# disanda/Deep-GAN-Encoders

Hardware: AMD Instinct MI355X
Metric: encoder-train images/sec (E_align_s2 step, StyleGAN2 FFHQ-1024) (higher is better)
Workload: dtype bf16; 1 GPU; E_align_s2 two-phase step, StyleGAN2-1024 G (train mode) + BE(startf=16, L=9) + LPIPS-VGG16 (seeded stand-in weights), batch 8/GPU; global_batch=8, img_size=1024, parallelism=dp1

## Files before the change

deep-gan-encoders_amd/_lib.py:

```python
import ctypes as C
import os

_HERE = os.path.dirname(os.path.abspath(__file__))
LIB_PATH = os.environ.get("DGE_LIB_PATH", os.path.join(_HERE, "libdge_hip.so"))


class DgeError(RuntimeError):
    pass


class ConvDesc(C.Structure):
    _fields_ = [
        ("x", C.c_void_p), ("w_packed", C.c_void_p), ("y", C.c_void_p), ("addend", C.c_void_p), ("dot_src", C.c_void_p),
        ("in_scale", C.c_void_p), ("in_shift", C.c_void_p), ("out_scale", C.c_void_p),
        ("bias", C.c_void_p), ("noise", C.c_void_p), ("noise_w", C.c_void_p), ("stats", C.c_void_p),
        ("B", C.c_int), ("H", C.c_int), ("W", C.c_int), ("Cin", C.c_int), ("Cout", C.c_int),
        ("ksize", C.c_int), ("up", C.c_int), ("in_s2d", C.c_int), ("noise_batch", C.c_int), ("noise_w_per_channel", C.c_int),
        ("act", C.c_int), ("bias_scale", C.c_float), ("gain", C.c_float), ("add_scale", C.c_float),
        ("dtype", C.c_int), ("in_up2", C.c_int), ("in_relu", C.c_int), ("stats_slots", C.c_int), ("w_layout", C.c_int),
        ("prep", C.c_int), ("prep_gain", C.c_float), ("prep_noise", C.c_void_p), ("prep_ns", C.c_void_p), ("prep_noise_batch", C.c_int),
        ("prep_stats", C.c_void_p), ("mask_relu", C.c_int), ("in_t2d", C.c_int),
        ("rgb_w", C.c_void_p), ("rgb_style", C.c_void_p), ("rgb_bias", C.c_void_p), ("rgb_out", C.c_void_p), ("rgb_wscale", C.c_float),
        ("rgb_skip_y", C.c_int), ("pool_out", C.c_int), ("pool_mask", C.c_void_p),
        ("prefetch_w", C.c_void_p), ("prefetch_ntot", C.c_int), ("prefetch_cin", C.c_int), ("in_bwd_coef", C.c_void_p),
# ... 37 lines not shown
    "dge_torgb_bwd_prep": [_P, _P, _P, _P, _P, _P, _I, _P, _P, _P, _I, _I, _I, _F, _F, _I, _P],
    "dge_demod_bwd_prep": [_P, _I, _P, _P, _P, _I, _I, _F, _P],
    "dge_sum_slots": [_P, _P, _I, _I, _I, _P],
    "dge_sum_slots_planar": [_P, _P, _I, _I, _I, _P],
    "dge_set_deterministic": [_I],
    "dge_get_deterministic": [],
    "dge_packed_n": [_I],
    "dge_pack_conv_weight": [_P, _P, _I, _I, _I, _I, _I, _F, _P],
    "dge_pack_conv_weights_multi": [_P, _P, _I, _I, _P],
    "dge_pack_desc_bytes": [],
    "dge_weight_sumsq": [_P, _P, _I, _I, _I, _F, _P],
    "dge_linear": [_P, _I, _P, _P, _P, _I, _I, _I, _I, _F, _F, _F, _I, _F, _I, _P],
    "dge_pixelnorm": [_P, _P, _I, _I, _F, _P],
    "dge_truncation": [_P, _P, _P, _I, _I, _I, _F, _I, _I, _P],
    "dge_torgb": [_P, _P, _P, _P, _P, _P, _I, _I, _I, _I, _F, _I, _P],
    "dge_conv_rgb_supported": [_I, _I, _I, _I, _I, _I, _I],
    "dge_conv_in_bwd_supported": [_I, _I, _I, _I, _I, _I, _I],
    "dge_conv_in_bwd_fromrgb_supported": [_I, _I, _I, _I, _I, _I, _I],
    "dge_conv_in_bwd_x_supported": [_I, _I, _I, _I, _I, _I, _I],
    "dge_conv_pool_supported": [_I, _I, _I, _I, _I, _I, _I],
    "dge_rgb_upsample_add": [_P, _P, _I, _I, _I, _P],
    "dge_nchw_to_nhwc": [_P, _P, _I, _I, _I, _I, _I, _P],
    "dge_nhwc_to_nchw": [_P, _P, _I, _I, _I, _I, _P],
    "dge_fromrgb": [_P, _P, _P, _P, _P, _I, _I, _I, _I, _P],
    "dge_fromrgb2": [_P, _P, _P, _P, _P, _P, _I, _I, _I, _I, _P],
    "dge_stats_finalize": [_P, _P, _P, _P, _I, _I, _I, _F, _P],
    "dge_stats_finalize_slots": [_P, _I, _P, _P, _P, _I, _I, _I, _F, _P],
    "dge_blend": [_P, _P, _P, _P, _P, _P, _I, _I, _I, _I, _I, _F, _F, _I, _P],
    "dge_loss_reduce": [_P, _P, _P, _I, _I, _I, _I, _I, _I, _I, _I, _P],
    "dge_crop_pool": [_P, _P, _I, _I, _I, _I, _I, _I, _I, _I, _P],
    "dge_ssim_fwd": [_P, _P, _P, _P, _I, _I, _I, _P],
    "dge_ssim_box7": [_P, _P, _P, _I, _I, _I, _F, _F, _F, _P],
    "dge_ssim_bwd": [_P, _P, _P, _P, _I, _I, _I, _F, _I, _P],
    "dge_space_loss_finalize": [_P, _P, _P, _P, _F, _F, _I, _P],
    "dge_space_loss_bwd": [_P, _P, _P, _P, _P, _I, _I, _I, _I, _I, _I, _I, _I, _F, _F, _I, _P],
    "dge_axpy_scalar": [_P, _P, _P, C.c_long, _F, _I, _P],
    "dge_lreq_adam_multi": [_I, _P, _P, _P, _P, _P, _F, _F, _P, _P, _P],
    "dge_modconv_bwd_prep": [_P, _P, _P, _P, _P, _P, _I, _I, _I, _I, _F, _I, _P],
    "dge_demod_bwd": [_P, _P, _P, _P, _P, _I, _I, _F, _P],
    "dge_linear_t": [_P, _I, _I, _P, _P, _P, _I, _I, _I, _I, _I, _F, _I, _P],
    "dge_torgb_bwd": [_P, _P, _P, _P, _P, _P, _I, _I, _I, _F, _I, _P],
    "dge_up2_bwd": [_P, _P, _I, _I, _I, _P],
    "dge_conv_wgrad": [_P, _P, _P, _P, _P, _I, _I, _I, _I, _I, _I, _I, _P],
    "dge_act_bwd": [_P, _P, _P, _P, _P, _I, _I, _I, _I, _I, _I, _F, _F, _I, _P],
    "dge_in_bwd_coef": [_P, _P, _P, _P, _P, _P, _I, _I, _I, _P],
    "dge_in_bwd_coef_slots": [_P, _I, _P, _P, _P, _P, _P, _I, _I, _I, _P],
    "dge_in_bwd": [_P, _P, _P, _P, _P, _P, _P, _I, _I, _I, _I, _I, _F, _I, _I, _P],
    "dge_chan_sum": [_P, _P, _I, _I, _I, _F, _I, _P],
    "dge_fromrgb_bwd": [_P, _P, _P, _P, _I, _I, _I, _I, _P],
    "dge_head_entry_size": [],
    "dge_heads_bwd": [_P, _I, _I, _P, _I, _P, _P, _P, _P, _I, _I, _P],
    "dge_dense_wgrad": [_P, _I, _P, _I, _P, _P, _I, _I, _I, _I, _P],
    "dge_lpips_prep": [_P, _P, _I, _I, _I, _P, _P, _I, _P],
    "dge_lpips_prep_bwd": [_P, _P, _I, _I, _I, _P, _F, _I, _I, _P],
    "dge_maxpool2": [_P, _P, _I, _I, _I, _I, _I, _P],
    "dge_maxpool2_bwd": [_P, _P, _P, _P, _I, _I, _I, _I, _I, _P],
    "dge_lpips_head": [_P, _P, _P, _P, _I, _I, _I, _F, _I, _P],
    "dge_mean": [_P, _P, _I, _P],
    "dge_blur_noise_act": [_P, _P, _P, _P, _P, _P, _I, _I, _I, _I, _I, _I, _I, _I, _P],
    "dge_affine_compose": [_P, _P, _P, _P, _P, _I, _I, _P],
    "dge_lerp_layers": [_P, _P, _I, _P, _P, _I, _I, _I, _P],
    "dge_linear_rows": [_P, _I, _P, _P, _P, _P, _P, _P, _I, _I, _I, _F, _F, _F, _P],
    "dge_demod_rows": [_P, _P, _P, _P, _P, _P, _P, _P, _I, _I, _F, _P],
    "dge_fromrgb_dgrad": [_P, _P, _P, _P, _I, _I, _I, _I, _P],
    "dge_nearest_up2": [_P, _P, _I, _I, _I, _I, _F, _I, _P],
    "dge_sg1_in_bwd_coef": [_P, _P, _P, _P, _P, _P, _I, _I, _I, _P],
# ... 93 lines not shown
```

deep-gan-encoders_amd/csrc/loss_kernels.hip:

```cpp
#include "common.h"
#include "../../include/dge_hip.h"

struct Crop { int H, W, y0, x0, h, w; };

__device__ __forceinline__ void block_atomic_sums(float* vals, int n, float* out, float* red) {
    const int lane = threadIdx.x & 63, wave = threadIdx.x >> 6;
    for (int i = 0; i < n; i++) {
        const float s = wave_sum(vals[i]);
        if (lane == 0) red[i * 4 + wave] = s;
    }
    __syncthreads();
    if (det_on()) {
        const int nslots = gridDim.x;
        float* slot = det_slot(0, 1, blockIdx.x, nslots, 8);
        if (threadIdx.x < n) slot[threadIdx.x] = red[threadIdx.x * 4] + red[threadIdx.x * 4 + 1] + red[threadIdx.x * 4 + 2] + red[threadIdx.x * 4 + 3];
        if (det_arrive_wg(0, nslots)) {
            __shared__ float dred[16];
            for (int i = 0; i < n; i++) {
                const float t = det_total_wg(0, nslots, 8, i, dred);
                if (threadIdx.x == 0) out[i] += t;
            }
        }
        return;
    }
// ... 12 lines not shown
        float ma = -INFINITY, mb = -INFINITY;
        for (int c = 0; c < C; c++) {
            const float av = a[off + c * plane], bv = b[off + c * plane];
            const float d = av - bv;
            v[0] += d * d; v[1] += av * bv; v[2] += av * av; v[3] += bv * bv; v[4] += av; v[5] += bv;
            ma = fmaxf(ma, av); mb = fmaxf(mb, bv);
        }
        float sa = 0.f, sb = 0.f;
        for (int c = 0; c < C; c++) { sa += __expf(a[off + c * plane] - ma); sb += __expf(b[off + c * plane] - mb); }
        const float lsa = __logf(sa) + ma, lsb = __logf(sb) + mb;
        for (int c = 0; c < C; c++) {
            const float la = a[off + c * plane] - lsa, lb = b[off + c * plane] - lsb;
            v[6] += __expf(la) * (la - lb);
        }
    }
    block_atomic_sums(v, 7, sums, red);
}

__global__ void crop_pool_kernel(const float* __restrict__ src, float* __restrict__ dst, int BC, Crop cr, int k) {
    const int oh = cr.h / k, ow = cr.w / k;
    const long n = (long)BC * oh * ow;
    const long idx = blockIdx.x * 256L + threadIdx.x;
    if (idx >= n) return;
    const int x = idx % ow; const long r = idx / ow; const int y = r % oh; const int bc = r / oh;
    const float* p = src + (size_t)bc * cr.H * cr.W + (size_t)(cr.y0 + y * k) * cr.W + cr.x0 + x * k;
    float s = 0.f;
    for (int i = 0; i < k; i++)
        for (int j = 0; j < k; j++) s += p[(size_t)i * cr.W + j];
    dst[idx] = s / (float)(k * k);
}

struct Gauss11 { float g[11]; };

__global__ __launch_bounds__(256) void ssim_fwd_kernel(const float* __restrict__ a, const float* __restrict__ b,
                                                        float* __restrict__ ssim_sum, float* __restrict__ dmap,
                                                        int BC, int h, int w, Gauss11 G) {
    __shared__ float ta[26][27], tb[26][27];
    __shared__ float red[4];
    const int bc = blockIdx.z, x0 = blockIdx.x * 16, y0 = blockIdx.y * 16;
    const float* pa = a + (size_t)bc * h * w; const float* pb = b + (size_t)bc * h * w;
    for (int i = threadIdx.x; i < 26 * 26; i += 256) {
        const int ty = i / 26, tx = i % 26, gy = y0 + ty - 5, gx = x0 + tx - 5;
        const bool in = gy >= 0 && gy < h && gx >= 0 && gx < w;
        ta[ty][tx] = in ? pa[(size_t)gy * w + gx] : 0.f;
        tb[ty][tx] = in ? pb[(size_t)gy * w + gx] : 0.f;
    }
    __syncthreads();
    const int lx = threadIdx.x % 16, ly = threadIdx.x / 16, gx = x0 + lx, gy = y0 + ly;
    float S = 0.f;
    if (gx < w && gy < h) {
        float mu1 = 0, mu2 = 0, e11 = 0, e22 = 0, e12 = 0;
        for (int i = 0; i < 11; i++)
            for (int j = 0; j < 11; j++) {
                const float wgt = G.g[i] * G.g[j];
                const float av = ta[ly + i][lx + j], bv = tb[ly + i][lx + j];
                mu1 += wgt * av; mu2 += wgt * bv; e11 += wgt * av * av; e22 += wgt * bv * bv; e12 += wgt * av * bv;
            }
        const float C1 = 1e-4f, C2 = 9e-4f;
        const float s11 = e11 - mu1 * mu1, s22 = e22 - mu2 * mu2, s12 = e12 - mu1 * mu2;
        const float A1 = 2 * mu1 * mu2 + C1, A2 = 2 * s12 + C2, B1 = mu1 * mu1 + mu2 * mu2 + C1, B2 = s11 + s22 + C2;
        const float inv = 1.f / (B1 * B2);
        S = A1 * A2 * inv;
        if (dmap) {
            const size_t n = (size_t)BC * h * w, o = (size_t)bc * h * w + (size_t)gy * w + gx;
            dmap[o] = (2 * mu1 * A2 - 2 * mu1 * A1) * inv - S * (2 * mu2 / B1 - 2 * mu2 / B2);
            dmap[n + o] = -S / B2;
            dmap[2 * n + o] = 2 * A1 * inv;
        }
    }
    S = wave_sum(S);
    if ((threadIdx.x & 63) == 0) red[threadIdx.x >> 6] = S;
    __syncthreads();
    if (det_on()) {
        const int nslots = gridDim.x * gridDim.y * gridDim.z;
        const int sl = blockIdx.x + gridDim.x * (blockIdx.y + gridDim.y * blockIdx.z);
        float* slot = det_slot(0, 1, sl, nslots, 1);
        if (threadIdx.x == 0) slot[0] = red[0] + red[1] + red[2] + red[3];
        if (det_arrive_wg(0, nslots)) {
            __shared__ float dred[16];
            const float t = det_total_wg(0, nslots, 1, 0, dred);
            if (threadIdx.x == 0) ssim_sum[0] += t;
        }
        return;
    }
    if (threadIdx.x == 0) atomicAdd(ssim_sum + ((blockIdx.x + blockIdx.y * 7 + blockIdx.z * 13) & 31), red[0] + red[1] + red[2] + red[3]);
}

__global__ __launch_bounds__(256) void ssim_bwd_kernel(const float* __restrict__ a, const float* __restrict__ b,
                                                        const float* __restrict__ dmap, float* __restrict__ g,
                                                        int BC, int h, int w, Gauss11 G, float scale, int accumulate) {
    __shared__ float t0[26][27], t1[26][27], t2[26][27];
    const int bc = blockIdx.z, x0 = blockIdx.x * 16, y0 = blockIdx.y * 16;
    const size_t n = (size_t)BC * h * w, po = (size_t)bc * h * w;
    for (int i = threadIdx.x; i < 26 * 26; i += 256) {
        const int ty = i / 26, tx = i % 26, gy = y0 + ty - 5, gx = x0 + tx - 5;
        const bool in = gy >= 0 && gy < h && gx >= 0 && gx < w;
        const size_t o = po + (size_t)gy * w + gx;
        t0[ty][tx] = in ? dmap[o] : 0.f; t1[ty][tx] = in ? dmap[n + o] : 0.f; t2[ty][tx] = in ? dmap[2 * n + o] : 0.f;
    }
    __syncthreads();
    const int lx = threadIdx.x % 16, ly = threadIdx.x / 16, gx = x0 + lx, gy = y0 + ly;
    if (gx >= w || gy >= h) return;
    float f0 = 0, f1 = 0, f2 = 0;
    for (int i = 0; i < 11; i++)
        for (int j = 0; j < 11; j++) {
            const float wgt = G.g[i] * G.g[j];
            f0 += wgt * t0[ly + i][lx + j]; f1 += wgt * t1[ly + i][lx + j]; f2 += wgt * t2[ly + i][lx + j];
        }
    const size_t o = po + (size_t)gy * w + gx;
    const float v = scale * (f0 + 2.f * b[o] * f1 + a[o] * f2);
    g[o] = accumulate ? g[o] + v : v;
}

__global__ void space_loss_finalize_kernel(const float* __restrict__ sums, const float* __restrict__ ssim_sum,
                                           const float* __restrict__ lpips, float* __restrict__ out, float n, float n_pooled,
                                           int image_space) {
    if (threadIdx.x != 0 || blockIdx.x != 0) return;
    const float mse = sums[0] / n;
    const float cosv = 1.f - sums[1] / (sqrtf(sums[2]) * sqrtf(sums[3]));
    const float ma = sums[4] / n, mb = sums[5] / n;
    const float va = fmaxf((sums[2] - n * ma * ma) / (n - 1.f), 0.f), vb = fmaxf((sums[3] - n * mb * mb) / (n - 1.f), 0.f);
    const float dm = ma - mb, ds = sqrtf(va) - sqrtf(vb);
    float kl = sums[6] / n;
    if (isnan(kl)) kl = 0.f;
    if (isinf(kl)) kl = 1.f;
    float ssim_tot = 0.f;
    if (image_space) for (int k = 0; k < 32; k++) ssim_tot += ssim_sum[k];
    const float ssim_l = image_space ? 1.f - ssim_tot / n_pooled : 0.f;
    const float lp = (image_space && lpips) ? lpips[0] : 0.f;
    out[0] = 5.f * mse + 3.f * cosv + ssim_l + 2.f * lp;
    out[1] = mse; out[2] = dm * dm; out[3] = ds * ds; out[4] = kl; out[5] = cosv; out[6] = ssim_l; out[7] = lp;
}

__global__ void space_loss_bwd_kernel(const float* __restrict__ a, const float* __restrict__ b,
                                      const float* __restrict__ sums, const float* __restrict__ gp, float* __restrict__ g,
                                      int BC, Crop cr, int k, float n, float wgt, int accumulate) {
    const long tot = (long)BC * cr.h * cr.w;
    const long idx = blockIdx.x * 256L + threadIdx.x;
    if (idx >= tot) return;
    const int x = idx % cr.w; const long r = idx / cr.w; const int y = r % cr.h; const int bc = r / cr.h;
    const size_t off = (size_t)bc * cr.H * cr.W + (size_t)(cr.y0 + y) * cr.W + cr.x0 + x;
    const float na = sqrtf(sums[2]), nb = sqrtf(sums[3]);
    const float av = a[off], bv = b[off];
    float v = 10.f * (bv - av) / n + 3.f * (-av / (na * nb) + sums[1] * bv / (na * nb * nb * nb));
// ... 410 lines not shown
        const float inv = 1.f / 49.f, cn = 49.f / 48.f;
        const float ux = sx * inv, uy = sy * inv;
        const float vx = cn * (sxx * inv - ux * ux), vy = cn * (syy * inv - uy * uy), vxy = cn * (sxy * inv - ux * uy);
        const float C1 = (0.01f * R) * (0.01f * R), C2 = (0.03f * R) * (0.03f * R);
        S = ((2 * ux * uy + C1) * (2 * vxy + C2)) / ((ux * ux + uy * uy + C1) * (vx + vy + C2));
    }
    S = wave_sum(S);
    if ((threadIdx.x & 63) == 0) red[threadIdx.x >> 6] = S;
    __syncthreads();
    if (det_on()) {
        const int nslots = gridDim.x * gridDim.y, sl = blockIdx.x + gridDim.x * blockIdx.y;
        float* slot = det_slot(bc, gridDim.z, sl, nslots, 1);
        if (threadIdx.x == 0) slot[0] = red[0] + red[1] + red[2] + red[3];
        if (det_arrive_wg(bc, nslots)) {
            __shared__ float dred[16];
            const float t = det_total_wg(bc, nslots, 1, 0, dred);
            if (threadIdx.x == 0) sums[bc] += t;
        }
        return;
    }
    if (threadIdx.x == 0) atomicAdd(sums + bc, red[0] + red[1] + red[2] + red[3]);
}

extern "C" int dge_ssim_box7(const float* a, const float* b, float* sums, int BC, int h, int w, float scale, float shift, float data_range,
                             hipStream_t s) {
    DGE_CHECK(BC >= 1 && h >= 7 && w >= 7 && data_range > 0.f, "ssim_box7: planes must be at least 7x7 (got %dx%d)", h, w);
    hipLaunchKernelGGL(ssim_box7_kernel, dim3((w - 6 + 15) / 16, (h - 6 + 15) / 16, BC), dim3(256), 0, s, a, b, sums, h, w, scale, shift,
                       data_range);
    DGE_LAUNCH_CHECK("ssim_box7");
    return 0;
}

extern "C" int dge_ssim_fwd(const float* a, const float* b, float* ssim_sum, float* dmap, int BC, int h, int w, hipStream_t s) {
    hipLaunchKernelGGL(ssim_fwd_kernel, dim3((w + 15) / 16, (h + 15) / 16, BC), dim3(256), 0, s, a, b, ssim_sum, dmap, BC, h, w, gauss11());
    DGE_LAUNCH_CHECK("ssim_fwd");
    return 0;
}

extern "C" int dge_ssim_bwd(const float* a, const float* b, const float* dmap, float* g, int BC, int h, int w, float scale,
                            int accumulate, hipStream_t s) {
    hipLaunchKernelGGL(ssim_bwd_kernel, dim3((w + 15) / 16, (h + 15) / 16, BC), dim3(256), 0, s, a, b, dmap, g, BC, h, w, gauss11(), scale, accumulate);
    DGE_LAUNCH_CHECK("ssim_bwd");
    return 0;
}

extern "C" int dge_space_loss_finalize(const float* sums7, const float* ssim_sum, const float* lpips, float* out8, float n,
                                       float n_pooled, int image_space, hipStream_t s) {
    hipLaunchKernelGGL(space_loss_finalize_kernel, dim3(1), dim3(64), 0, s, sums7, ssim_sum, lpips, out8, n, n_pooled, image_space);
    DGE_LAUNCH_CHECK("space_loss_finalize");
    return 0;
}

extern "C" int dge_space_loss_bwd(const float* a, const float* b, const float* sums7, const float* g_pooled, float* g,
                                  int BC, int H, int W, int y0, int x0, int h, int w, int k, float n, float weight,
                                  int accumulate, hipStream_t s) {
    const long tot = (long)BC * h * w;
    hipLaunchKernelGGL(space_loss_bwd_kernel, dim3((unsigned)((tot + 255) / 256)), dim3(256), 0, s, a, b, sums7, g_pooled, g, BC,
                       mk(H, W, y0, x0, h, w), k, n, weight, accumulate);
    DGE_LAUNCH_CHECK("space_loss_bwd");
    return 0;
}

extern "C" int dge_axpy_scalar(const float* x, const float* scalar, float* y, long n, float extra, int accumulate, hipStream_t s) {
    hipLaunchKernelGGL(axpy_scalar_kernel, dim3((unsigned)((n + 255) / 256)), dim3(256), 0, s, x, scalar, y, n, extra, accumulate);
    DGE_LAUNCH_CHECK("axpy_scalar");
    return 0;
}
```

deep-gan-encoders_amd/losses.py:

```python
import contextlib
import os

import torch

from . import ops
from ._lib import lib, check
from .collectives import all_reduce
from .ops import _f32, _p, _stream


class GlobalBatch:

    def __init__(self, world):
        self.world = world

    def reduce(self, t):
        all_reduce(t)
        return t


def _pool_factor(h):
    k = 1
    while h > 256:
        h //= 2
        k *= 2
    return k


def attention_windows(H, W):
    oy, ox = H // 8 + H // 32, W // 8 + W // 32
    return [(0, 0, H, W), (0, W // 8, H, W - 2 * (W // 8)), (oy, ox, H - 2 * oy, W - 2 * ox)]


_PK = 48


def _window_reduce(a, b, win, image_space, lpips_model, need_grad, pk, world):
    B, Cc, H, W = a.shape
    y0, x0, h, w = win
    dev = a.device
    L = lib()
    slots = ops.zeros((16, 8), dev)
    check(L.dge_loss_reduce(_f32(a), _f32(b), _p(slots), B, Cc, H, W, y0, x0, h, w, _stream()), "dge_loss_reduce")
    ops._sum_over_batch(slots, pk[0:8])
    st = dict(win=win, pk=pk, k=1, npool=1.0, n=float(B * Cc * h * w) * world, lp=None, ap=None)
    if image_space:
        k = _pool_factor(h)
        hp, wp = h // k, w // k
        ap = torch.empty((B, Cc, hp, wp), dtype=torch.float32, device=dev)
        bp = torch.empty_like(ap)
        check(L.dge_crop_pool(_f32(a), _p(ap), B * Cc, H, W, y0, x0, h, w, k, _stream()), "dge_crop_pool")
        check(L.dge_crop_pool(_f32(b), _p(bp), B * Cc, H, W, y0, x0, h, w, k, _stream()), "dge_crop_pool")
        dmap = torch.empty((3, B, Cc, hp, wp), dtype=torch.float32, device=dev) if need_grad else None
        check(L.dge_ssim_fwd(_p(ap), _p(bp), _p(pk[8:40]), _p(dmap), B * Cc, hp, wp, _stream()), "dge_ssim_fwd")
        st.update(k=k, npool=float(B * Cc * hp * wp) * world, ap=ap, bp=bp, dmap=dmap, g_lp=None)
        if lpips_model is not None:
            lp, st["g_lp"] = lpips_model.value_and_grad(ap, bp, need_grad=need_grad)
            if world > 1:
                check(L.dge_axpy_scalar(_p(lp), None, _p(pk[40:41]), 1, 1.0 / world, 0, _stream()), "dge_axpy_scalar")
                lp = pk[40:41]
            st["lp"] = lp
    return st


def _window_finish(a, b, st, image_space, weight, g_out, accumulate, world):
    B, Cc, H, W = a.shape
    y0, x0, h, w = st["win"]
    dev = a.device
    L = lib()
    pk = st["pk"]
    out8 = torch.empty(8, dtype=torch.float32, device=dev)
    gp = None
    if image_space and g_out is not None:
        bp = st["bp"]
        gp = torch.empty_like(bp)
        check(L.dge_ssim_bwd(_p(st["ap"]), _p(bp), _p(st["dmap"]), _p(gp), B * Cc, bp.shape[2], bp.shape[3], -1.0 / st["npool"], 0,
                             _stream()), "dge_ssim_bwd")
        if st["g_lp"] is not None:
            check(L.dge_axpy_scalar(_p(st["g_lp"]), None, _p(gp), gp.numel(), 2.0 / world, 1, _stream()), "dge_axpy_scalar")
    check(L.dge_space_loss_finalize(_p(pk[0:8]), _p(pk[8:40]) if image_space else None, _p(st["lp"]), _p(out8), st["n"], st["npool"],
                                    1 if image_space else 0, _stream()), "dge_space_loss_finalize")
    if g_out is not None:
        check(L.dge_space_loss_bwd(_f32(a), _f32(b), _p(pk[0:8]), _p(gp), _p(g_out), B * Cc, H, W, y0, x0, h, w, st["k"], st["n"],
                                   float(weight), 1 if accumulate else 0, _stream()), "dge_space_loss_bwd")
    return out8


def _space_loss_windows(a, b, wins, image_space, lpips_model, weights, g_outs, accumulate, gb=None):
    world = gb.world if gb is not None else 1
    pack = ops.zeros((len(wins), _PK), a.device)
    sts = [_window_reduce(a, b, win, image_space, lpips_model, g_outs[i] is not None, pack[i], world) for i, win in enumerate(wins)]
    if gb is not None:
        gb.reduce(pack)
    return [_window_finish(a, b, st, image_space, weights[i], g_outs[i], accumulate, world) for i, st in enumerate(sts)]


_WINDOW_STREAMS = os.environ.get("DGE_WINDOW_STREAMS", "1") != "0" and os.environ.get("DGE_SIDE_STREAMS", "1") != "0"
_SIDE = {}


def _side_streams(dev, n):
    key = (dev.index if dev.index is not None else torch.cuda.current_device())
    have = _SIDE.setdefault(key, [])
    while len(have) < n:
        have.append(torch.cuda.Stream(device=dev))
    return have[:n]


def _space_loss_windows3(a, b, wins, lpips_model, weights, g, need, gb=None, g_split=None):
    import ctypes as C
# ... 3 lines not shown
    world = gb.world if gb is not None else 1
    nw = len(wins)
    pack = ops.zeros((nw, _PK), dev)
    slots = ops.zeros((nw, 16, 8), dev)
    wflat = (C.c_int * (4 * nw))(*[int(v) for win in wins for v in win])
    check(L.dge_loss_reduce3(_f32(a), _f32(b), _p(slots), B, Cc, H, W, wflat, nw, _stream()), "dge_loss_reduce3")
    sums = ops.DeferredSums()
    for i in range(nw):
        sums.add(slots[i].view(16, 8, 1), pack[i, 0:8])
    sums.flush()
    ks = [_pool_factor(win[2]) for win in wins]
    aps = [torch.empty((B, Cc, win[2] // k, win[3] // k), dtype=torch.float32, device=dev) for win, k in zip(wins, ks)]
    bps = [torch.empty_like(t) for t in aps]
    srcs = (C.c_void_p * (2 * nw))(*([a.data_ptr()] * nw + [b.data_ptr()] * nw))
    dsts = (C.c_void_p * (2 * nw))(*([t.data_ptr() for t in aps] + [t.data_ptr() for t in bps]))
    w2 = (C.c_int * (8 * nw))(*([int(v) for win in wins for v in win] * 2))
    k2 = (C.c_int * (2 * nw))(*(ks * 2))
    check(L.dge_crop_pool_multi(srcs, dsts, w2, k2, 2 * nw, B * Cc, H, W, _stream()), "dge_crop_pool_multi")
    sts = []
    main = torch.cuda.current_stream(dev) if dev.type == "cuda" else None
    fork = (main is not None and lpips_model is not None and nw > 1 and _WINDOW_STREAMS and not ops.is_deterministic()
            and getattr(lpips_model, "_streams_warm", False)
            and (B * H * W >= (4 << 20) or torch.cuda.is_current_stream_capturing()))
    side = _side_streams(dev, nw - 1) if fork else []
    for i, win in enumerate(wins):
        y0, x0, h, w = win
        ap, bp, k = aps[i], bps[i], ks[i]
        hp, wp = h // k, w // k
        ng = (g is not None or g_split is not None) and need[i]
        strm = side[i - 1] if (fork and i > 0) else None
        if strm is not None:
            strm.wait_stream(main)
        with (torch.cuda.stream(strm) if strm is not None else contextlib.nullcontext()):
            dmap = torch.empty((3, B, Cc, hp, wp), dtype=torch.float32, device=dev) if ng else None
            check(L.dge_ssim_fwd(_p(ap), _p(bp), _p(pack[i, 8:40]), _p(dmap), B * Cc, hp, wp, _stream()), "dge_ssim_fwd")
            st = dict(win=win, pk=pack[i], k=k, npool=float(B * Cc * hp * wp) * world, n=float(B * Cc * h * w) * world, ap=ap, bp=bp,
                      dmap=dmap, g_lp=None, lp=None, ng=ng)
            if lpips_model is not None:
                lp, st["g_lp"] = lpips_model.value_and_grad(ap, bp, need_grad=ng)
                if world > 1:
                    check(L.dge_axpy_scalar(_p(lp), None, _p(pack[i, 40:41]), 1, 1.0 / world, 0, _stream()), "dge_axpy_scalar")
                    lp = pack[i, 40:41]
                st["lp"] = lp
            st["gp"] = None
            if ng:
                gp = torch.empty_like(bp)
                check(L.dge_ssim_bwd(_p(ap), _p(bp), _p(dmap), _p(gp), B * Cc, hp, wp, -1.0 / st["npool"], 0, _stream()), "dge_ssim_bwd")
                if st["g_lp"] is not None:
                    check(L.dge_axpy_scalar(_p(st["g_lp"]), None, _p(gp), gp.numel(), 2.0 / world, 1, _stream()), "dge_axpy_scalar")
                st["gp"] = gp
        if strm is not None:
            for t in (dmap, st["g_lp"], st["lp"], st["gp"]):
                if t is not None:
                    t.record_stream(main)
        sts.append(st)
    for strm in side:
        main.wait_stream(strm)
    if lpips_model is not None:
        lpips_model._streams_warm = True
    if gb is not None:
        gb.reduce(pack)
    outs, gps = [], []
    for i, st in enumerate(sts):
        gps.append(st["gp"])
        out8 = torch.empty(8, dtype=torch.float32, device=dev)
        check(L.dge_space_loss_finalize(_p(pack[i, 0:8]), _p(pack[i, 8:40]), _p(st["lp"]), _p(out8), st["n"], st["npool"], 1, _stream()),
              "dge_space_loss_finalize")
        outs.append(out8)
    if g is not None:
        sp = (C.c_void_p * nw)(*[pack[i, 0:8].data_ptr() for i in range(nw)])
        gpp = (C.c_void_p * nw)(*[(t.data_ptr() if t is not None else None) for t in gps])
        nn = (C.c_float * nw)(*[st["n"] for st in sts])
        ww = (C.c_float * nw)(*[float(weights[i]) if sts[i]["ng"] else 0.0 for i in range(nw)])
        kk = (C.c_int * nw)(*ks)
        check(L.dge_space_loss_bwd3(_f32(a), _f32(b), sp, gpp, _p(g), B * Cc, H, W, wflat, kk, nn, ww, nw, _stream()), "dge_space_loss_bwd3")
    if g_split is not None:
        _bwd_split(a, b, wins, [pack[i, 0:8] for i in range(nw)], gps, ks, [st["n"] for st in sts],
                   [float(weights[i]) if sts[i]["ng"] else 0.0 for i in range(nw)], g_split)
    return outs


def _bwd_split(a, b, wins, sums, gps, ks, ns, wts, outs):
    import ctypes as C
    if all(t is None for t in outs):
        return
    B, Cc, H, W = a.shape
    nw = len(wins)
    ptrs = lambda ts: (C.c_void_p * nw)(*[(t.data_ptr() if t is not None else None) for t in ts])
    wflat = (C.c_int * (4 * nw))(*[int(v) for win in wins for v in win])
    check(lib().dge_space_loss_bwd_split(_f32(a), _f32(b), ptrs(sums), ptrs(gps), ptrs(outs), B * Cc, H, W, wflat, (C.c_int * nw)(*ks),
                                         (C.c_float * nw)(*ns), (C.c_float * nw)(*wts), nw, _stream()), "dge_space_loss_bwd_split")
    ops.log_kernel()


def _space_loss_windows_split(a, b, wins, lpips_model, weights, g_split, gb=None):
    B, Cc = a.shape[:2]
    L = lib()
    world = gb.world if gb is not None else 1
    pack = ops.zeros((len(wins), _PK), a.device)
    sts = [_window_reduce(a, b, win, True, lpips_model, g_split[i] is not None, pack[i], world) for i, win in enumerate(wins)]
    if gb is not None:
        gb.reduce(pack)
    outs, gps = [], []
    for i, st in enumerate(sts):
        gp = None
        if g_split[i] is not None:
            bp = st["bp"]
            gp = torch.empty_like(bp)
            check(L.dge_ssim_bwd(_p(st["ap"]), _p(bp), _p(st["dmap"]), _p(gp), B * Cc, bp.shape[2], bp.shape[3], -1.0 / st["npool"], 0,
                                 _stream()), "dge_ssim_bwd")
            if st["g_lp"] is not None:
                check(L.dge_axpy_scalar(_p(st["g_lp"]), None, _p(gp), gp.numel(), 2.0 / world, 1, _stream()), "dge_axpy_scalar")
        gps.append(gp)
        outs.append(_window_finish(a, b, st, True, weights[i], None, False, world))
    _bwd_split(a, b, wins, [pack[i, 0:8] for i in range(len(wins))], gps, [st["k"] for st in sts], [st["n"] for st in sts],
               [float(weights[i]) if g_split[i] is not None else 0.0 for i in range(len(wins))], g_split)
    return outs


def _space_loss_window(a, b, win, image_space, lpips_model, weight, g_out, accumulate, gb=None):
    return _space_loss_windows(a, b, [win], image_space, lpips_model, [weight], [g_out], accumulate, gb)[0]


class _ScaledGrad(torch.autograd.Function):

    @staticmethod
    def forward(ctx, b, loss, g):
        ctx.save_for_backward(g)
        return loss.clone()

    @staticmethod
    def backward(ctx, go):
        (g,) = ctx.saved_tensors
        out = torch.empty_like(g)
        check(lib().dge_axpy_scalar(_p(g), _p(go.contiguous().float()), _p(out), g.numel(), 1.0, 0, _stream()), "dge_axpy_scalar")
        return out, None, None


class _ScaledGrad2(torch.autograd.Function):

    @staticmethod
    def forward(ctx, a, b, loss, ga, gb):
        ctx.save_for_backward(ga, gb)
# ... 80 lines not shown
```

include/dge_hip.h:

```cpp
#ifndef DGE_HIP_H
#define DGE_HIP_H
#include <stddef.h>
#ifdef __cplusplus
extern "C" {
#endif

typedef struct ihipStream_t* dge_stream_t;

#define DGE_DTYPE_F32 0
#define DGE_DTYPE_BF16 1
#define DGE_ACT_LINEAR 0
#define DGE_ACT_LRELU02 1
#define DGE_ACT_RELU_ 2
#define DGE_LIN_RSQRT 3
#define DGE_PACK_FWD 0
#define DGE_PACK_UPFOLD 1
#define DGE_PACK_DGRAD 2
#define DGE_PACK_UPFOLD_DGRAD 3
#define DGE_PACK_SG1_UP 4
#define DGE_PACK_SG1_UP_DGRAD 5
#define DGE_PACK_UPT2D_DGRAD 6

const char* dge_last_error(void);
int dge_version(void);
// ... 82 lines not shown
                   int w_is_wp, dge_stream_t stream);

int dge_torgb(const void* x, const float* wrgb, const float* style, const float* bias, const float* prev, float* img,
              int B, int H, int W, int cin, float wscale, int dtype, dge_stream_t stream);

int dge_conv_rgb_supported(int B, int H, int W, int Cin, int Cout, int ksize, int dtype);
int dge_conv_in_bwd_supported(int B, int H, int W, int Cin, int Cout, int ksize, int dtype);
int dge_conv_in_bwd_fromrgb_supported(int B, int H, int W, int Cin, int Cout, int ksize, int dtype);
int dge_conv_in_bwd_x_supported(int B, int H, int W, int Cin, int Cout, int ksize, int dtype);
int dge_conv_pool_supported(int B, int H, int W, int Cin, int Cout, int ksize, int dtype);
int dge_rgb_upsample_add(float* img, const float* prev, int BC, int H, int W, dge_stream_t stream);
int dge_nchw_to_nhwc(const float* src, void* dst, int B, int C, int HW, int src_B, int dtype, dge_stream_t stream);
int dge_nhwc_to_nchw(const void* src, float* dst, int B, int C, int HW, int dtype, dge_stream_t stream);

int dge_fromrgb(const float* img, const float* w, const float* bias, void* y, float* stats, int B, int HW, int C,
                int dtype, dge_stream_t stream);
int dge_fromrgb2(const float* img, const float* w, const float* bias, void* y, float* stats, float* img4, int B, int HW, int C,
                 int dtype, dge_stream_t stream);
int dge_stats_finalize(const float* stats, float* musig, float* sc, float* sh, int B, int C, int npix, float eps,
                       dge_stream_t stream);
int dge_stats_finalize_slots(const float* stats, int nslot, float* musig, float* sc, float* sh, int B, int C, int npix, float eps,
                             dge_stream_t stream);
int dge_blend(const void* x, const void* z, void* y, const float* sc, const float* sh, float* stats, int B, int OH,
              int OW, int C, int pool, float alpha, float beta, int dtype, dge_stream_t stream);

int dge_loss_reduce(const float* a, const float* b, float* sums7, int B, int C, int H, int W, int y0, int x0, int h, int w,
                    dge_stream_t stream);
int dge_crop_pool(const float* src, float* dst, int BC, int H, int W, int y0, int x0, int h, int w, int k, dge_stream_t stream);
int dge_ssim_fwd(const float* a, const float* b, float* ssim_sum, float* dmap, int BC, int h, int w, dge_stream_t stream);
int dge_ssim_box7(const float* a, const float* b, float* sums, int BC, int h, int w, float scale, float shift, float data_range,
                  dge_stream_t stream);
int dge_ssim_bwd(const float* a, const float* b, const float* dmap, float* g, int BC, int h, int w, float scale,
                 int accumulate, dge_stream_t stream);
int dge_space_loss_finalize(const float* sums7, const float* ssim_sum, const float* lpips, float* out8, float n,
                            float n_pooled, int image_space, dge_stream_t stream);
int dge_space_loss_bwd(const float* a, const float* b, const float* sums7, const float* g_pooled, float* g, int BC, int H,
                       int W, int y0, int x0, int h, int w, int k, float n, float weight, int accumulate, dge_stream_t stream);
int dge_loss_reduce3(const float* a, const float* b, float* sums, int B, int C, int H, int W, const int* wins, int nwin, dge_stream_t stream);
int dge_crop_pool_multi(const float* const* src, float* const* dst, const int* wins, const int* ks, int n, int BC, int H, int W,
                        dge_stream_t stream);
int dge_space_loss_bwd3(const float* a, const float* b, const float* const* sums7, const float* const* g_pooled, float* g, int BC, int H,
                        int W, const int* wins, const int* ks, const float* n, const float* weight, int nwin, dge_stream_t stream);
int dge_space_loss_bwd_split(const float* a, const float* b, const float* const* sums7, const float* const* g_pooled, float* const* g,
                             int BC, int H, int W, const int* wins, const int* ks, const float* n, const float* weight, int nwin,
                             dge_stream_t stream);
int dge_axpy_scalar(const float* x, const float* scalar, float* y, long n, float extra, int accumulate, dge_stream_t stream);

int dge_lreq_adam_multi(int ntensors, float* const* host_p, const float* const* host_g, float* const* host_v,
                        const long* host_n, const float* host_step, float beta2, float eps, const float* gscale,
                        const float* step_mult, dge_stream_t stream);

int dge_modconv_bwd_prep(const void* gx, const void* x, const float* d, const float* noise, void* gy, float* R, int B,
                         int HW, int C, int noise_batch, float gain, int dtype, dge_stream_t stream);
int dge_demod_bwd(const float* R, const float* d, const float* bias, const float* noise_strength, float* t, int B, int C,
                  float bscale, dge_stream_t stream);
int dge_linear_t(const float* x, int ldx, int incx, const float* w, const float* mul, float* y, int ldy, int incy, int B,
                 int O, int K, float scale, int accumulate, dge_stream_t stream);
int dge_torgb_bwd(const float* gimg, const void* x, const float* wrgb, const float* style, void* gx, float* gs, int B,
                  int HW, int C, float wscale, int dtype, dge_stream_t stream);
int dge_torgb_bwd_prep(const float* gimg, const void* x, const float* wrgb, const float* style, const float* noise,
                       const float* noise_strength, int noise_batch, void* gz, float* gs, float* P, int B, int HW, int C,
                       float wscale, float gain, int dtype, dge_stream_t stream);
int dge_fir_t2d(const void* g, const float* scale, void* z, int B, int H, int W, int C, int dtype, dge_stream_t stream);
typedef struct dge_s2_grad_entry {
    const float* P; const float* st; const float* d; const float* s; const float* bias; const float* wsq;
    const float* gs; const float* wstyle;
// ... 168 lines not shown
```

Measured before the change: 374.7 images/sec.

## Fuse SSIM forward and backward into one separable-filter kernel without dmap

Replaces the direct 11x11 SSIM window sums with separable row and column Gaussian passes on larger 32x32 tiles. Adds a fused forward+backward kernel that computes the SSIM partial maps on a halo region in shared memory and immediately convolves them for the gradient, so the three-plane dmap is never written to or reread from global memory and one launch is dropped. The cost is redundant halo computation, heavier shared-memory use (possibly lower occupancy), and the gradient now being computed eagerly in the forward phase.

```diff
diff --git a/deep-gan-encoders_amd/_lib.py b/deep-gan-encoders_amd/_lib.py
--- a/deep-gan-encoders_amd/_lib.py
+++ b/deep-gan-encoders_amd/_lib.py
@@ -93,6 +93,7 @@
     "dge_ssim_fwd": [_P, _P, _P, _P, _I, _I, _I, _P],
     "dge_ssim_box7": [_P, _P, _P, _I, _I, _I, _F, _F, _F, _P],
     "dge_ssim_bwd": [_P, _P, _P, _P, _I, _I, _I, _F, _I, _P],
+    "dge_ssim_fwd_bwd": [_P, _P, _P, _P, _I, _I, _I, _F, _I, _P],
     "dge_space_loss_finalize": [_P, _P, _P, _P, _F, _F, _I, _P],
     "dge_space_loss_bwd": [_P, _P, _P, _P, _P, _I, _I, _I, _I, _I, _I, _I, _I, _F, _F, _I, _P],
     "dge_axpy_scalar": [_P, _P, _P, C.c_long, _F, _I, _P],
diff --git a/deep-gan-encoders_amd/csrc/loss_kernels.hip b/deep-gan-encoders_amd/csrc/loss_kernels.hip
--- a/deep-gan-encoders_amd/csrc/loss_kernels.hip
+++ b/deep-gan-encoders_amd/csrc/loss_kernels.hip
@@ -68,42 +68,95 @@
 
 struct Gauss11 { float g[11]; };
 
-__global__ __launch_bounds__(256) void ssim_fwd_kernel(const float* __restrict__ a, const float* __restrict__ b,
-                                                        float* __restrict__ ssim_sum, float* __restrict__ dmap,
-                                                        int BC, int h, int w, Gauss11 G) {
-    __shared__ float ta[26][27], tb[26][27];
-    __shared__ float red[4];
-    const int bc = blockIdx.z, x0 = blockIdx.x * 16, y0 = blockIdx.y * 16;
-    const float* pa = a + (size_t)bc * h * w; const float* pb = b + (size_t)bc * h * w;
-    for (int i = threadIdx.x; i < 26 * 26; i += 256) {
-        const int ty = i / 26, tx = i % 26, gy = y0 + ty - 5, gx = x0 + tx - 5;
+constexpr int ST = 32;
+constexpr int SH1 = ST + 10;
+constexpr int SH2 = ST + 20;
+
+template <int IH, int IW, int IS>
+__device__ __forceinline__ void ssim_stage_ab(const float* __restrict__ pa, const float* __restrict__ pb, float* ta, float* tb,
+                                              int oy, int ox, int h, int w) {
+    for (int i = threadIdx.x; i < IH * IW; i += 256) {
+        const int ty = i / IW, tx = i % IW, gy = oy + ty, gx = ox + tx;
         const bool in = gy >= 0 && gy < h && gx >= 0 && gx < w;
-        ta[ty][tx] = in ? pa[(size_t)gy * w + gx] : 0.f;
-        tb[ty][tx] = in ? pb[(size_t)gy * w + gx] : 0.f;
-    }
-    __syncthreads();
-    const int lx = threadIdx.x % 16, ly = threadIdx.x / 16, gx = x0 + lx, gy = y0 + ly;
-    float S = 0.f;
-    if (gx < w && gy < h) {
-        float mu1 = 0, mu2 = 0, e11 = 0, e22 = 0, e12 = 0;
-        for (int i = 0; i < 11; i++)
+        ta[ty * IS + tx] = in ? pa[(size_t)gy * w + gx] : 0.f;
+        tb[ty * IS + tx] = in ? pb[(size_t)gy * w + gx] : 0.f;
+    }
+}
+
+template <int IH, int OW, int RW, int IS>
+__device__ __forceinline__ void ssim_row_pass_ab(const float* ta, const float* tb, float* R, const Gauss11& G) {
+    static_assert(OW % RW == 0, "row pass: whole groups");
+    for (int item = threadIdx.x; item < IH * (OW / RW); item += 256) {
+        const int y = item % IH, x = (item / IH) * RW;
+        float av[RW + 10], bv[RW + 10];
+#pragma unroll
+        for (int j = 0; j < RW + 10; j++) { av[j] = ta[y * IS + x + j]; bv[j] = tb[y * IS + x + j]; }
+#pragma unroll
+        for (int o = 0; o < RW; o++) {
+            float m1 = 0, m2 = 0, e11 = 0, e22 = 0, e12 = 0;
+#pragma unroll
             for (int j = 0; j < 11; j++) {
-                const float wgt = G.g[i] * G.g[j];
-                const float av = ta[ly + i][lx + j], bv = tb[ly + i][lx + j];
-                mu1 += wgt * av; mu2 += wgt * bv; e11 += wgt * av * av; e22 += wgt * bv * bv; e12 += wgt * av * bv;
-            }
-        const float C1 = 1e-4f, C2 = 9e-4f;
-        const float s11 = e11 - mu1 * mu1, s22 = e22 - mu2 * mu2, s12 = e12 - mu1 * mu2;
-        const float A1 = 2 * mu1 * mu2 + C1, A2 = 2 * s12 + C2, B1 = mu1 * mu1 + mu2 * mu2 + C1, B2 = s11 + s22 + C2;
-        const float inv = 1.f / (B1 * B2);
-        S = A1 * A2 * inv;
-        if (dmap) {
-            const size_t n = (size_t)BC * h * w, o = (size_t)bc * h * w + (size_t)gy * w + gx;
-            dmap[o] = (2 * mu1 * A2 - 2 * mu1 * A1) * inv - S * (2 * mu2 / B1 - 2 * mu2 / B2);
-            dmap[n + o] = -S / B2;
-            dmap[2 * n + o] = 2 * A1 * inv;
-        }
-    }
+                const float wa = G.g[j] * av[o + j], wb = G.g[j] * bv[o + j];
+                m1 += wa; m2 += wb; e11 += wa * av[o + j]; e22 += wb * bv[o + j]; e12 += wa * bv[o + j];
+            }
+            float* r = R + y * OW + x + o;
+            r[0] = m1; r[IH * OW] = m2; r[2 * IH * OW] = e11; r[3 * IH * OW] = e22; r[4 * IH * OW] = e12;
+        }
+    }
+}
+
+template <int IH, int OW, int RW, int IS>
+__device__ __forceinline__ void ssim_row_pass3(const float* P, float* R, const Gauss11& G) {
+    static_assert(OW % RW == 0, "row pass: whole groups");
+    for (int item = threadIdx.x; item < 3 * IH * (OW / RW); item += 256) {
+        const int y = item % IH, q = item / IH, x = (q % (OW / RW)) * RW, m = q / (OW / RW);
+        float v[RW + 10];
+#pragma unroll
+        for (int j = 0; j < RW + 10; j++) v[j] = P[(m * IH + y) * IS + x + j];
+#pragma unroll
+        for (int o = 0; o < RW; o++) {
+            float f = 0;
+#pragma unroll
+            for (int j = 0; j < 11; j++) f += G.g[j] * v[o + j];
+            R[(m * IH + y) * OW + x + o] = f;
+        }
+    }
+}
+
+template <int NM, int CR, int IH, int OW>
+__device__ __forceinline__ void ssim_col_pass(const float* R, int y, int x, const Gauss11& G, float (&acc)[CR][NM]) {
+#pragma unroll
+    for (int r = 0; r < CR; r++)
+#pragma unroll
+        for (int m = 0; m < NM; m++) acc[r][m] = 0.f;
+#pragma unroll
+    for (int i = 0; i < CR + 10; i++) {
+        float v[NM];
+#pragma unroll
+        for (int m = 0; m < NM; m++) v[m] = R[(m * IH + y + i) * OW + x];
+#pragma unroll
+        for (int r = 0; r < CR; r++)
+            if (i - r >= 0 && i - r < 11) {
+#pragma unroll
+                for (int m = 0; m < NM; m++) acc[r][m] += G.g[i - r] * v[m];
+            }
+    }
+}
+
+__device__ __forceinline__ float ssim_point(const float (&m)[5], float& d0, float& d1, float& d2) {
+    const float mu1 = m[0], mu2 = m[1], e11 = m[2], e22 = m[3], e12 = m[4];
+    const float C1 = 1e-4f, C2 = 9e-4f;
+    const float s11 = e11 - mu1 * mu1, s22 = e22 - mu2 * mu2, s12 = e12 - mu1 * mu2;
+    const float A1 = 2 * mu1 * mu2 + C1, A2 = 2 * s12 + C2, B1 = mu1 * mu1 + mu2 * mu2 + C1, B2 = s11 + s22 + C2;
+    const float inv = 1.f / (B1 * B2);
+    const float S = A1 * A2 * inv;
+    d0 = (2 * mu1 * A2 - 2 * mu1 * A1) * inv - S * (2 * mu2 / B1 - 2 * mu2 / B2);
+    d1 = -S / B2;
+    d2 = 2 * A1 * inv;
+    return S;
+}
+
+__device__ __forceinline__ void ssim_block_sum(float S, float* __restrict__ ssim_sum, float* red) {
     S = wave_sum(S);
     if ((threadIdx.x & 63) == 0) red[threadIdx.x >> 6] = S;
     __syncthreads();
@@ -122,30 +175,104 @@
     if (threadIdx.x == 0) atomicAdd(ssim_sum + ((blockIdx.x + blockIdx.y * 7 + blockIdx.z * 13) & 31), red[0] + red[1] + red[2] + red[3]);
 }
 
+__device__ __forceinline__ void ssim_grad_tile(const float* P, float* R, const float* __restrict__ pa, const float* __restrict__ pb,
+                                               float* __restrict__ pg, int y0, int x0, int h, int w, const Gauss11& G, float scale,
+                                               int accumulate) {
+    ssim_row_pass3<SH1, ST, 4, SH1 + 1>(P, R, G);
+    __syncthreads();
+    const int lx = threadIdx.x % ST, ly = (threadIdx.x / ST) * 4, gx = x0 + lx;
+    float f[4][3];
+    ssim_col_pass<3, 4, SH1, ST>(R, ly, lx, G, f);
+#pragma unroll
+    for (int r = 0; r < 4; r++) {
+        const int gy = y0 + ly + r;
+        if (gx < w && gy < h) {
+            const size_t o = (size_t)gy * w + gx;
+            const float v = scale * (f[r][0] + 2.f * pb[o] * f[r][1] + pa[o] * f[r][2]);
+            pg[o] = accumulate ? pg[o] + v : v;
+        }
+    }
+}
+
+__global__ __launch_bounds__(256) void ssim_fwd_kernel(const float* __restrict__ a, const float* __restrict__ b,
+                                                        float* __restrict__ ssim_sum, float* __restrict__ dmap,
+                                                        int BC, int h, int w, Gauss11 G) {
+    __shared__ float ta[SH1 * (SH1 + 1)], tb[SH1 * (SH1 + 1)], R[5 * SH1 * ST];
+    __shared__ float red[4];
+    const int bc = blockIdx.z, x0 = blockIdx.x * ST, y0 = blockIdx.y * ST;
+    ssim_stage_ab<SH1, SH1, SH1 + 1>(a + (size_t)bc * h * w, b + (size_t)bc * h * w, ta, tb, y0 - 5, x0 - 5, h, w);
+    __syncthreads();
+    ssim_row_pass_ab<SH1, ST, 4, SH1 + 1>(ta, tb, R, G);
+    __syncthreads();
+    const int lx = threadIdx.x % ST, ly = (threadIdx.x / ST) * 4, gx = x0 + lx;
+    float m[4][5];
+    ssim_col_pass<5, 4, SH1, ST>(R, ly, lx, G, m);
+    float S = 0.f;
+#pragma unroll
+    for (int r = 0; r < 4; r++) {
+        const int gy = y0 + ly + r;
+        if (gx < w && gy < h) {
+            float d0, d1, d2;
+            S += ssim_point(m[r], d0, d1, d2);
+            if (dmap) {
+                const size_t n = (size_t)BC * h * w, o = (size_t)bc * h * w + (size_t)gy * w + gx;
+                dmap[o] = d0; dmap[n + o] = d1; dmap[2 * n + o] = d2;
+            }
+        }
+    }
+    ssim_block_sum(S, ssim_sum, red);
+}
+
 __global__ __launch_bounds__(256) void ssim_bwd_kernel(const float* __restrict__ a, const float* __restrict__ b,
                                                         const float* __restrict__ dmap, float* __restrict__ g,
                                                         int BC, int h, int w, Gauss11 G, float scale, int accumulate) {
-    __shared__ float t0[26][27], t1[26][27], t2[26][27];
-    const int bc = blockIdx.z, x0 = blockIdx.x * 16, y0 = blockIdx.y * 16;
+    __shared__ float P[3 * SH1 * (SH1 + 1)], R[3 * SH1 * ST];
+    const int bc = blockIdx.z, x0 = blockIdx.x * ST, y0 = blockIdx.y * ST;
     const size_t n = (size_t)BC * h * w, po = (size_t)bc * h * w;
-    for (int i = threadIdx.x; i < 26 * 26; i += 256) {
-        const int ty = i / 26, tx = i % 26, gy = y0 + ty - 5, gx = x0 + tx - 5;
+    for (int i = threadIdx.x; i < SH1 * SH1; i += 256) {
+        const int ty = i / SH1, tx = i % SH1, gy = y0 + ty - 5, gx = x0 + tx - 5;
         const bool in = gy >= 0 && gy < h && gx >= 0 && gx < w;
         const size_t o = po + (size_t)gy * w + gx;
-        t0[ty][tx] = in ? dmap[o] : 0.f; t1[ty][tx] = in ? dmap[n + o] : 0.f; t2[ty][tx] = in ? dmap[2 * n + o] : 0.f;
-    }
-    __syncthreads();
-    const int lx = threadIdx.x % 16, ly = threadIdx.x / 16, gx = x0 + lx, gy = y0 + ly;
-    if (gx >= w || gy >= h) return;
-    float f0 = 0, f1 = 0, f2 = 0;
-    for (int i = 0; i < 11; i++)
-        for (int j = 0; j < 11; j++) {
-            const float wgt = G.g[i] * G.g[j];
-            f0 += wgt * t0[ly + i][lx + j]; f1 += wgt * t1[ly + i][lx + j]; f2 += wgt * t2[ly + i][lx + j];
-        }
-    const size_t o = po + (size_t)gy * w + gx;
-    const float v = scale * (f0 + 2.f * b[o] * f1 + a[o] * f2);
-    g[o] = accumulate ? g[o] + v : v;
+        float* p = P + ty * (SH1 + 1) + tx;
+        p[0] = in ? dmap[o] : 0.f; p[SH1 * (SH1 + 1)] = in ? dmap[n + o] : 0.f; p[2 * SH1 * (SH1 + 1)] = in ? dmap[2 * n + o] : 0.f;
+    }
+    __syncthreads();
+    ssim_grad_tile(P, R, a + po, b + po, g + po, y0, x0, h, w, G, scale, accumulate);
+}
+
+__global__ __launch_bounds__(256) void ssim_fwd_bwd_kernel(const float* __restrict__ a, const float* __restrict__ b,
+                                                            float* __restrict__ ssim_sum, float* __restrict__ g,
+                                                            int BC, int h, int w, Gauss11 G, float scale, int accumulate) {
+    constexpr int TS = SH2 + 1, PS = SH1 + 1;
+    __shared__ float T[2 * SH2 * TS];
+    __shared__ float R[5 * SH2 * SH1];
+    __shared__ float red[4];
+    static_assert(3 * SH1 * PS <= 2 * SH2 * TS, "the partial maps reuse the staged tiles");
+    const int bc = blockIdx.z, x0 = blockIdx.x * ST, y0 = blockIdx.y * ST;
+    const size_t po = (size_t)bc * h * w;
+    ssim_stage_ab<SH2, SH2, TS>(a + po, b + po, T, T + SH2 * TS, y0 - 10, x0 - 10, h, w);
+    __syncthreads();
+    ssim_row_pass_ab<SH2, SH1, 6, TS>(T, T + SH2 * TS, R, G);
+    __syncthreads();
+    float S = 0.f;
+    if (threadIdx.x < SH1 * 6) {
+        const int lx = threadIdx.x % SH1, ly = (threadIdx.x / SH1) * 7, gx = x0 - 5 + lx;
+        float m[7][5];
+        ssim_col_pass<5, 7, SH2, SH1>(R, ly, lx, G, m);
+#pragma unroll
+        for (int r = 0; r < 7; r++) {
+            const int gy = y0 - 5 + ly + r;
+            const bool in = gx >= 0 && gx < w && gy >= 0 && gy < h;
+            float d0, d1, d2;
+            const float s = ssim_point(m[r], d0, d1, d2);
+            if (in && lx >= 5 && lx < 5 + ST && ly + r >= 5 && ly + r < 5 + ST) S += s;
+            float* p = T + (ly + r) * PS + lx;
+            p[0] = in ? d0 : 0.f; p[SH1 * PS] = in ? d1 : 0.f; p[2 * SH1 * PS] = in ? d2 : 0.f;
+        }
+    }
+    __syncthreads();
+    ssim_grad_tile(T, R, a + po, b + po, g + po, y0, x0, h, w, G, scale, accumulate);
+    ssim_block_sum(S, ssim_sum, red);
 }
 
 __global__ void space_loss_finalize_kernel(const float* __restrict__ sums, const float* __restrict__ ssim_sum,
@@ -622,15 +749,26 @@
 }
 
 extern "C" int dge_ssim_fwd(const float* a, const float* b, float* ssim_sum, float* dmap, int BC, int h, int w, hipStream_t s) {
-    hipLaunchKernelGGL(ssim_fwd_kernel, dim3((w + 15) / 16, (h + 15) / 16, BC), dim3(256), 0, s, a, b, ssim_sum, dmap, BC, h, w, gauss11());
+    hipLaunchKernelGGL(ssim_fwd_kernel, dim3((w + ST - 1) / ST, (h + ST - 1) / ST, BC), dim3(256), 0, s, a, b, ssim_sum, dmap, BC, h, w, gauss11());
     DGE_LAUNCH_CHECK("ssim_fwd");
     return 0;
 }
 
 extern "C" int dge_ssim_bwd(const float* a, const float* b, const float* dmap, float* g, int BC, int h, int w, float scale,
                             int accumulate, hipStream_t s) {
-    hipLaunchKernelGGL(ssim_bwd_kernel, dim3((w + 15) / 16, (h + 15) / 16, BC), dim3(256), 0, s, a, b, dmap, g, BC, h, w, gauss11(), scale, accumulate);
+    hipLaunchKernelGGL(ssim_bwd_kernel, dim3((w + ST - 1) / ST, (h + ST - 1) / ST, BC), dim3(256), 0, s, a, b, dmap, g, BC, h, w, gauss11(), scale, accumulate);
     DGE_LAUNCH_CHECK("ssim_bwd");
+    return 0;
+}
+
+extern "C" int dge_ssim_fwd_bwd(const float* a, const float* b, float* ssim_sum, float* g, int BC, int h, int w, float scale,
+                                int accumulate, hipStream_t s) {
+    DGE_CHECK(a && b && ssim_sum && g && BC >= 1 && BC <= 65535 && h >= 1 && w >= 1, "ssim_fwd_bwd: bad arguments");
+    const dim3 grid((w + ST - 1) / ST, (h + ST - 1) / ST, BC);
+    DGE_CHECK(grid.y <= 65535 && dge_det_fits(1, (long long)grid.x * grid.y * grid.z, 1),
+              "ssim_fwd_bwd: %d planes of %dx%d do not fit the launch (or the deterministic-mode workspace)", BC, h, w);
+    hipLaunchKernelGGL(ssim_fwd_bwd_kernel, grid, dim3(256), 0, s, a, b, ssim_sum, g, BC, h, w, gauss11(), scale, accumulate);
+    DGE_LAUNCH_CHECK("ssim_fwd_bwd");
     return 0;
 }
 
diff --git a/deep-gan-encoders_amd/losses.py b/deep-gan-encoders_amd/losses.py
--- a/deep-gan-encoders_amd/losses.py
+++ b/deep-gan-encoders_amd/losses.py
@@ -33,6 +33,17 @@
 
 
 _PK = 48
+
+
+def _ssim_value_and_grad(ap, bp, ssim_slots, npool, need_grad):
+    B, Cc, hp, wp = ap.shape
+    L = lib()
+    if not need_grad:
+        check(L.dge_ssim_fwd(_p(ap), _p(bp), _p(ssim_slots), None, B * Cc, hp, wp, _stream()), "dge_ssim_fwd")
+        return None
+    gp = torch.empty_like(bp)
+    check(L.dge_ssim_fwd_bwd(_p(ap), _p(bp), _p(ssim_slots), _p(gp), B * Cc, hp, wp, -1.0 / npool, 0, _stream()), "dge_ssim_fwd_bwd")
+    return gp
 
 
 def _window_reduce(a, b, win, image_space, lpips_model, need_grad, pk, world):
@@ -51,9 +62,8 @@
         bp = torch.empty_like(ap)
         check(L.dge_crop_pool(_f32(a), _p(ap), B * Cc, H, W, y0, x0, h, w, k, _stream()), "dge_crop_pool")
         check(L.dge_crop_pool(_f32(b), _p(bp), B * Cc, H, W, y0, x0, h, w, k, _stream()), "dge_crop_pool")
-        dmap = torch.empty((3, B, Cc, hp, wp), dtype=torch.float32, device=dev) if need_grad else None
-        check(L.dge_ssim_fwd(_p(ap), _p(bp), _p(pk[8:40]), _p(dmap), B * Cc, hp, wp, _stream()), "dge_ssim_fwd")
-        st.update(k=k, npool=float(B * Cc * hp * wp) * world, ap=ap, bp=bp, dmap=dmap, g_lp=None)
+        st.update(k=k, npool=float(B * Cc * hp * wp) * world, ap=ap, bp=bp, gp=None, g_lp=None)
+        st["gp"] = _ssim_value_and_grad(ap, bp, pk[8:40], st["npool"], need_grad)
         if lpips_model is not None:
             lp, st["g_lp"] = lpips_model.value_and_grad(ap, bp, need_grad=need_grad)
             if world > 1:
@@ -72,10 +82,7 @@
     out8 = torch.empty(8, dtype=torch.float32, device=dev)
     gp = None
     if image_space and g_out is not None:
-        bp = st["bp"]
-        gp = torch.empty_like(bp)
-        check(L.dge_ssim_bwd(_p(st["ap"]), _p(bp), _p(st["dmap"]), _p(gp), B * Cc, bp.shape[2], bp.shape[3], -1.0 / st["npool"], 0,
-                             _stream()), "dge_ssim_bwd")
+        gp = st["gp"]
         if st["g_lp"] is not None:
             check(L.dge_axpy_scalar(_p(st["g_lp"]), None, _p(gp), gp.numel(), 2.0 / world, 1, _stream()), "dge_axpy_scalar")
     check(L.dge_space_loss_finalize(_p(pk[0:8]), _p(pk[8:40]) if image_space else None, _p(st["lp"]), _p(out8), st["n"], st["npool"],
@@ -145,25 +152,19 @@
         if strm is not None:
             strm.wait_stream(main)
         with (torch.cuda.stream(strm) if strm is not None else contextlib.nullcontext()):
-            dmap = torch.empty((3, B, Cc, hp, wp), dtype=torch.float32, device=dev) if ng else None
-            check(L.dge_ssim_fwd(_p(ap), _p(bp), _p(pack[i, 8:40]), _p(dmap), B * Cc, hp, wp, _stream()), "dge_ssim_fwd")
             st = dict(win=win, pk=pack[i], k=k, npool=float(B * Cc * hp * wp) * world, n=float(B * Cc * h * w) * world, ap=ap, bp=bp,
-                      dmap=dmap, g_lp=None, lp=None, ng=ng)
+                      g_lp=None, lp=None, ng=ng)
+            gp = st["gp"] = _ssim_value_and_grad(ap, bp, pack[i, 8:40], st["npool"], ng)
             if lpips_model is not None:
                 lp, st["g_lp"] = lpips_model.value_and_grad(ap, bp, need_grad=ng)
                 if world > 1:
                     check(L.dge_axpy_scalar(_p(lp), None, _p(pack[i, 40:41]), 1, 1.0 / world, 0, _stream()), "dge_axpy_scalar")
                     lp = pack[i, 40:41]
                 st["lp"] = lp
-            st["gp"] = None
-            if ng:
-                gp = torch.empty_like(bp)
-                check(L.dge_ssim_bwd(_p(ap), _p(bp), _p(dmap), _p(gp), B * Cc, hp, wp, -1.0 / st["npool"], 0, _stream()), "dge_ssim_bwd")
-                if st["g_lp"] is not None:
-                    check(L.dge_axpy_scalar(_p(st["g_lp"]), None, _p(gp), gp.numel(), 2.0 / world, 1, _stream()), "dge_axpy_scalar")
-                st["gp"] = gp
+            if ng and st["g_lp"] is not None:
+                check(L.dge_axpy_scalar(_p(st["g_lp"]), None, _p(gp), gp.numel(), 2.0 / world, 1, _stream()), "dge_axpy_scalar")
         if strm is not None:
-            for t in (dmap, st["g_lp"], st["lp"], st["gp"]):
+            for t in (st["g_lp"], st["lp"], st["gp"]):
                 if t is not None:
                     t.record_stream(main)
         sts.append(st)
@@ -218,10 +219,7 @@
     for i, st in enumerate(sts):
         gp = None
         if g_split[i] is not None:
-            bp = st["bp"]
-            gp = torch.empty_like(bp)
-            check(L.dge_ssim_bwd(_p(st["ap"]), _p(bp), _p(st["dmap"]), _p(gp), B * Cc, bp.shape[2], bp.shape[3], -1.0 / st["npool"], 0,
-                                 _stream()), "dge_ssim_bwd")
+            gp = st["gp"]
             if st["g_lp"] is not None:
                 check(L.dge_axpy_scalar(_p(st["g_lp"]), None, _p(gp), gp.numel(), 2.0 / world, 1, _stream()), "dge_axpy_scalar")
         gps.append(gp)
diff --git a/include/dge_hip.h b/include/dge_hip.h
--- a/include/dge_hip.h
+++ b/include/dge_hip.h
@@ -138,6 +138,8 @@
                   dge_stream_t stream);
 int dge_ssim_bwd(const float* a, const float* b, const float* dmap, float* g, int BC, int h, int w, float scale,
                  int accumulate, dge_stream_t stream);
+int dge_ssim_fwd_bwd(const float* a, const float* b, float* ssim_sum, float* g, int BC, int h, int w, float scale,
+                     int accumulate, dge_stream_t stream);
 int dge_space_loss_finalize(const float* sums7, const float* ssim_sum, const float* lpips, float* out8, float n,
                             float n_pooled, int image_space, dge_stream_t stream);
 int dge_space_loss_bwd(const float* a, const float* b, const float* sums7, const float* g_pooled, float* g, int BC, int H,
```

After: 377.4 images/sec, median of 6. No clear change (+0.7%).
